# speedinghzl/CCNet

Measured on NVIDIA B200. Metric: cca_fwd_bwd_pixels_per_s, higher is better.
Workload: dtype f32

## Files before the change

ccnet_b200/csrc/cca_tc_bwd.cu:

```cuda
#include "cca_items.cuh"
#include "cca_tc_common.cuh"

namespace cca {
namespace {
using namespace tc;

constexpr int kTmemCols = 512;
constexpr int kTmemO = 256, kTmemQK = 384;
constexpr int kRegsSoft = 104, kRegsEpi = 128, kRegsConvB = 48;
static_assert(reg_pool_ok(kRegsSoft, kRegsEpi, kRegsConvB), "setmaxnreg pool");
constexpr int kZeroBuf = 2048;

struct BwdParams {
    ItemSpace sp;
    int C, Cq;
    long npix;
    const float *lse;
    float *delta;
    unsigned int *zdone;
    unsigned int *ddone;
    int delta_mode;
    int out_mode;
    unsigned int *cdone;
    int lag;
    int hints;
    uint8_t *dq, *dk, *dv;
    long sb_q, sb_v;
    long share_q, share_v;
    int ahead;
    long long *dbg;
};

#ifdef CCA_TIMELINE
#define CCA_STAMP(role)                                                                          \
    do {                                                                                         \
        if (p.dbg && blockIdx.x == 0 && dbg_n < 512) p.dbg[(role) * 512 + dbg_n++] = clock64();  \
    } while (0)
#else
#define CCA_STAMP(role) do { } while (0)
#endif

template <int LK, bool BF> struct BwdSmem {
    using T = Tiles<LK, BF>;
    static constexpr int kNLd = BF ? 6 : 5;
    static constexpr int off_ld = 0;
    static constexpr int kNOut = BF ? 3 : 1;
    static constexpr int off_out = off_ld + kNLd * T::kSlot;
    static constexpr int off_p = off_out + kNOut * T::kSlot;
    static constexpr int off_tail = off_p + T::kP + (16 - LK / 8) * T::kPlane;
    static constexpr int off_zero = off_tail + (128 - LK) * 16 + 256;
    static constexpr int off_dpart = off_zero + kZeroBuf;
    static constexpr int off_bar = off_dpart + 2048 + 32;
    static constexpr int kBytes = off_bar + 8 * 48 + 32;
    static_assert(kBytes <= 232448, "shared memory budget");
};

enum { B_LD_FULL = 0, B_LD_EMPTY = 6, B_OP_FULL = 12, B_S_FULL = 18, B_S_EMPTY = 20, B_P_FULL = 22,
       B_P_EMPTY = 23, B_O_FULL = 24, B_O_EMPTY = 26, B_OUT_FULL = 28, B_STAGED = 29, B_DP_FULL = 30, B_DS_FULL = 31,
       B_DELTA_FULL = 32, B_DELTA_EMPTY = 33, B_OUT_FREE = 34, B_STAGED_W = 37, B_QK_FULL = 43, B_QK_EMPTY = 45,
       B_COUNT = 47 };

__device__ __forceinline__ bool calc_delta(const BwdParams &p, const Item &it) { return p.delta_mode == 0 || (it.col && it.ik == 0); }

template <int LK, bool BF>
__device__ __forceinline__ float convert_dot(uint8_t *dslot, const uint8_t *oslot, int t, uint64_t *o_empty, unsigned int *o_cnt)
{
    using T = Tiles<LK, BF>;
    const int grp = t >> 8, r = t & 127, hq = (t >> 7) & 1;
    const int rr = r < LK ? r : LK - 1;
    const int sw = rr & 7;
    float acc = 0.f;
    auto group_sync_and_release = [&]() {
        if (grp == 0) asm volatile("bar.sync 1, 256;" ::: "memory");
        else asm volatile("bar.sync 3, 256;" ::: "memory");
        if ((t & 255) == 0 && atomicAdd(o_cnt, 1u) == 1u) {
            *o_cnt = 0u;
            mbar_arrive(o_empty);
        }
    };
    if constexpr (BF) {
        const uint8_t *a = dslot + rr * 128, *b = oslot + rr * 128;
#pragma unroll
        for (int i = 0; i < 2; ++i) {
            const int j = (grp * 2 + hq) * 2 + i;
            const uint4 x = *reinterpret_cast<const uint4 *>(a + ((j ^ sw) * 16));
            const uint4 y = *reinterpret_cast<const uint4 *>(b + ((j ^ sw) * 16));
            const uint32_t xw[4] = {x.x, x.y, x.z, x.w}, yw[4] = {y.x, y.y, y.z, y.w};
#pragma unroll
            for (int e = 0; e < 4; ++e) acc += bf_lo(xw[e]) * bf_lo(yw[e]) + bf_hi(xw[e]) * bf_hi(yw[e]);
        }
        group_sync_and_release();
    } else {
        float4 raw[4];
        uint8_t *box = dslot + grp * T::kTile;
        const uint8_t *src = box + rr * 128;
        const uint8_t *osrc = oslot + grp * T::kTile + rr * 128;
#pragma unroll
        for (int j = 0; j < 4; ++j) raw[j] = *reinterpret_cast<const float4 *>(src + (((hq * 4 + j) ^ sw) * 16));
#pragma unroll
        for (int j = 0; j < 4; ++j) {
            const float4 o = *reinterpret_cast<const float4 *>(osrc + (((hq * 4 + j) ^ sw) * 16));
            acc += raw[j].x * o.x + raw[j].y * o.y + raw[j].z * o.z + raw[j].w * o.w;
        }
        group_sync_and_release();
        if (r < LK) {
            uint8_t *d = box + r * 16 + hq * 2 * T::kPStride;
#pragma unroll
            for (int j = 0; j < 2; ++j) {
                const float4 a = raw[2 * j], b = raw[2 * j + 1];
                const float v[8] = {a.x, a.y, a.z, a.w, b.x, b.y, b.z, b.w};
                uint4 hi, lo;
                split8(v, hi, lo);
                *reinterpret_cast<uint4 *>(d + j * T::kPStride) = hi;
                *reinterpret_cast<uint4 *>(d + j * T::kPStride + T::kLoOff) = lo;
            }
        }
    }
    return acc;
}

template <int LK, bool BF>
__global__ void __launch_bounds__(kThreads, 1)
cca_tc_bwd_kernel(const __grid_constant__ CUtensorMap mqc, const __grid_constant__ CUtensorMap mqr,
                  const __grid_constant__ CUtensorMap mkc, const __grid_constant__ CUtensorMap mkr,
                  const __grid_constant__ CUtensorMap mvc, const __grid_constant__ CUtensorMap mvr,
                  const __grid_constant__ CUtensorMap mdoc, const __grid_constant__ CUtensorMap mdor,
                  const __grid_constant__ CUtensorMap moc, const __grid_constant__ CUtensorMap mor,
                  const __grid_constant__ CUtensorMap mdqc, const __grid_constant__ CUtensorMap mdqr,
                  const __grid_constant__ CUtensorMap mdkc, const __grid_constant__ CUtensorMap mdkr,
                  const __grid_constant__ CUtensorMap mdvc, const __grid_constant__ CUtensorMap mdvr, BwdParams p)
{
    using T = Tiles<LK, BF>;
    using S = BwdSmem<LK, BF>;
    constexpr int TERMS = BF ? 1 : 3;
    constexpr int kNLd = S::kNLd;
    constexpr int kNOut = S::kNOut;
    extern __shared__ __align__(1024) uint8_t smem[];
    uint64_t *bars = reinterpret_cast<uint64_t *>(smem + S::off_bar);
    uint32_t *tmem_slot = reinterpret_cast<uint32_t *>(smem + S::off_bar + 8 * B_COUNT);
    float *dpart = reinterpret_cast<float *>(smem + S::off_dpart);
    unsigned int *o_cnt = reinterpret_cast<unsigned int *>(smem + S::off_dpart + 2048);
    const int tid = threadIdx.x, warp = tid >> 5, lane = tid & 31;
    const int NCH = p.C / kNC;
    const int KQ = p.Cq / 16;
    const int NO = NCH + 2;
    const int nk = p.sp.total > (int)blockIdx.x ? (p.sp.total - (int)blockIdx.x + (int)gridDim.x - 1) / (int)gridDim.x : 0;
    auto item_of = [&](int k) { return decode_item_order(p.sp, (int)blockIdx.x + k * (int)gridDim.x, p.lag); };

    if (tid == 0) {
        for (int i = 0; i < kNLd; ++i) {
            mbar_init(&bars[B_LD_FULL + i], 1); mbar_init(&bars[B_LD_EMPTY + i], 1); mbar_init(&bars[B_OP_FULL + i], kConvThreads);
        }
        for (int i = 0; i < 2; ++i) { mbar_init(&bars[B_O_FULL + i], 1); mbar_init(&bars[B_O_EMPTY + i], 128); }
        for (int i = 0; i < 3; ++i) { mbar_init(&bars[B_OUT_FREE + i], 1); mbar_init(&bars[B_STAGED_W + i], 128); mbar_init(&bars[B_STAGED_W + 3 + i], 128); }
        for (int i = 0; i < 2; ++i) { mbar_init(&bars[B_S_FULL + i], 1); mbar_init(&bars[B_S_EMPTY + i], 128); }
        for (int i = 0; i < 2; ++i) { mbar_init(&bars[B_QK_FULL + i], 1); mbar_init(&bars[B_QK_EMPTY + i], 128); }
        mbar_init(&bars[B_P_FULL], 128); mbar_init(&bars[B_P_EMPTY], 1);
        mbar_init(&bars[B_DP_FULL], 1);  mbar_init(&bars[B_DS_FULL], 128);
        mbar_init(&bars[B_DELTA_FULL], kConvThreads); mbar_init(&bars[B_DELTA_EMPTY], 128);
        fence_mbar_init();
        prefetch_tmap(&mqc); prefetch_tmap(&mqr); prefetch_tmap(&mkc); prefetch_tmap(&mkr); prefetch_tmap(&mvc); prefetch_tmap(&mvr);
        prefetch_tmap(&mdoc); prefetch_tmap(&mdor); prefetch_tmap(&moc); prefetch_tmap(&mor);
        prefetch_tmap(&mdqc); prefetch_tmap(&mdqr); prefetch_tmap(&mdkc); prefetch_tmap(&mdkr); prefetch_tmap(&mdvc); prefetch_tmap(&mdvr);
    }
    if (tid < kZeroBuf / 16) {
        reinterpret_cast<uint4 *>(smem + S::off_zero)[tid] = make_uint4(0, 0, 0, 0);
        fence_proxy_async();
    }
    if (tid < 8) o_cnt[tid] = 0u;
    if (warp == 0) tmem_alloc<kTmemCols>(tmem_slot);
    tc_fence_before();
    __syncthreads();
    tc_fence_after();
    const uint32_t tmem = *tmem_slot;

    if (warp >= kWarpProducer) {
        reg_dec<kRegsMisc>();
        if (warp == kWarpProducer) {
            if (lane == 0) {
                uint32_t g = 0;
                int dbg_n = 0;
                (void)dbg_n;
                const uint64_t pol_keep = l2_policy_evict_last(), pol_stream = l2_policy_evict_first();
                auto emit = [&](const CUtensorMap *mc, const CUtensorMap *mr, int c0, const Item &it, int start, bool last_use = false) {
                    const CUtensorMap *m = it.col ? mc : mr;
                    const int cw = it.col ? it.line : start, ch = it.col ? start : it.line;
                    const int slot = g % kNLd;
                    mbar_wait(&bars[B_LD_EMPTY + slot], ((g / kNLd) & 1) ^ 1);
                    CCA_STAMP(0);
                    uint8_t *dst = smem + S::off_ld + slot * T::kSlot;
                    mbar_expect_tx(&bars[B_LD_FULL + slot], T::kSlot);
                    if (p.hints == 1) {
                        const uint64_t pol = (is_producer(it) && !last_use) ? pol_keep : pol_stream;
                        tma_load_4d(dst, m, &bars[B_LD_FULL + slot], c0, cw, ch, it.b, pol);
                        if constexpr (!BF) tma_load_4d(dst + T::kTile, m, &bars[B_LD_FULL + slot], c0 + 32, cw, ch, it.b, pol);
                    } else {
                        tma_load_4d(dst, m, &bars[B_LD_FULL + slot], c0, cw, ch, it.b);
                        if constexpr (!BF) tma_load_4d(dst + T::kTile, m, &bars[B_LD_FULL + slot], c0 + 32, cw, ch, it.b);
                    }
                    ++g;
                };
                if (nk > 0) {
                    const Item it0 = item_of(0);
                    emit(&mqc, &mqr, 0, it0, it0.q0);
                    emit(&mkc, &mkr, 0, it0, it0.k0);
                }
                for (int k = 0; k < nk; ++k) {
                    const Item it = item_of(k);
                    const bool calc = calc_delta(p, it);
                    for (int n = 0; n < NCH; ++n) {
                        emit(&mvc, &mvr, n * kNC, it, it.k0);
                        emit(&mdoc, &mdor, n * kNC, it, it.q0);
                        if (calc) emit(&moc, &mor, n * kNC, it, it.q0, p.delta_mode == 1);
                    }
                    if (k + 1 < nk) {
                        const Item nx = item_of(k + 1);
                        emit(&mqc, &mqr, 0, nx, nx.q0);
                        emit(&mkc, &mkr, 0, nx, nx.k0);
                    }
                    emit(&mqc, &mqr, 0, it, it.q0);
                    emit(&mkc, &mkr, 0, it, it.k0);
                }
            }
        } else if (warp == kWarpMma) {
            const uint32_t id_kk_s = instr_desc(kFmtBF16, kFmtBF16, 128, LK, false, false);
            const uint32_t id_mn_mn = instr_desc(kFmtBF16, kFmtBF16, 128, kNC, true, true);
            const uint32_t id_k_mn = instr_desc(kFmtBF16, kFmtBF16, 128, kNC, false, true);
            const uint32_t pb = smem_u32(smem + S::off_p);
            const uint32_t LO8 = BF ? 0 : T::kLoOff, LOP = T::kPP * T::kPlane;
            uint32_t u = 0, oc = 0;
            int dbg_n = lane == 0 ? 0 : 512;
            (void)dbg_n;
            const uint32_t ld_base = smem_u32(smem + S::off_ld);
            auto opb = [&](uint32_t g) { return ld_base + (g % kNLd) * T::kSlot; };
            auto wait_op = [&](uint32_t g) { mbar_wait(&bars[B_OP_FULL + g % kNLd], (g / kNLd) & 1); };
            auto free_op = [&](uint32_t g) { commit_to(&bars[B_LD_EMPTY + g % kNLd]); };
            constexpr uint32_t KS_K = BF ? 32 : 2 * T::kPStride, LBO_K = BF ? 16 : T::kPStride, SBO_K = BF ? 1024 : 128;
            constexpr uint32_t KS_MN = BF ? 2048 : 256, LBO_MN = BF ? 16 : 128, SBO_MN = BF ? 1024 : T::kPStride;
            constexpr uint32_t LAY = BF ? kSw128 : 0;
            auto issue_s = [&](int k) {
                const uint32_t q = opb(u), kk = opb(u + 1);
                wait_op(u); wait_op(u + 1);
                mbar_wait(&bars[B_S_EMPTY + (k & 1)], ((k >> 1) & 1) ^ 1);
                tc_fence_after();
                const uint32_t d = tmem + (k & 1) * 128;
                for (int ks = 0; ks < KQ; ++ks) {
                    const uint32_t ao = ks * KS_K;
                    mma_split3<TERMS>(d, smem_desc(q + ao, LBO_K, SBO_K, LAY), smem_desc(q + LO8 + ao, LBO_K, SBO_K, LAY),
                                      smem_desc(kk + ao, LBO_K, SBO_K, LAY), smem_desc(kk + LO8 + ao, LBO_K, SBO_K, LAY), id_kk_s, ks > 0);
                }
                commit_to(&bars[B_S_FULL + (k & 1)]);
                free_op(u); free_op(u + 1);
                u += 2;
            };
            if (nk > 0) issue_s(0);
            for (int k = 0; k < nk; ++k) {
                const bool calc = calc_delta(p, item_of(k));
                CCA_STAMP(2);
                const uint32_t sdp = tmem + (k & 1) * 128;
                mbar_wait(&bars[B_P_FULL], k & 1);
                CCA_STAMP(2);
                for (int n = 0; n < NCH; ++n, u += calc ? 3 : 2, ++oc) {
                    const uint32_t vb = opb(u), db = opb(u + 1);
                    wait_op(u); wait_op(u + 1);
                    tc_fence_after();
                    mma_split3_loop<kNC / 16, TERMS>(sdp, db, db + LO8, KS_K, LBO_K, SBO_K,
                                                     vb, vb + LO8, KS_K, LBO_K, SBO_K, id_kk_s, n > 0, LAY, LAY);
                    free_op(u);
                    mbar_wait(&bars[B_O_EMPTY + (oc & 1)], ((oc >> 1) & 1) ^ 1);
                    tc_fence_after();
                    mma_split3_loop<LK / 16, TERMS>(tmem + kTmemO + (oc & 1) * kNC, pb, pb + LOP, 256, 128, T::kPlane,
                                                    db, db + LO8, KS_MN, LBO_MN, SBO_MN, id_mn_mn, false, 0, LAY);
                    commit_to(&bars[B_O_FULL + (oc & 1)]);
                    free_op(u + 1);
                    CCA_STAMP(2);
                }
                commit_to(&bars[B_DP_FULL]);
                if (k + 1 < nk) issue_s(k + 1);
                mbar_wait(&bars[B_DS_FULL], k & 1);
                CCA_STAMP(2);
                {
                    const uint32_t q = opb(u), kk = opb(u + 1);
                    wait_op(u); wait_op(u + 1);
                    mbar_wait(&bars[B_QK_EMPTY + 0], (k & 1) ^ 1);
                    mbar_wait(&bars[B_QK_EMPTY + 1], (k & 1) ^ 1);
                    tc_fence_after();
                    mma_split3_loop<LK / 16, TERMS>(tmem + kTmemQK, pb, pb + LOP, 2 * T::kPlane, T::kPlane, 128,
                                                    kk, kk + LO8, KS_MN, LBO_MN, SBO_MN, id_k_mn, false, 0, LAY);
                    commit_to(&bars[B_QK_FULL + 0]);
                    free_op(u + 1);
                    mma_split3_loop<LK / 16, TERMS>(tmem + kTmemQK + kNC, pb, pb + LOP, 256, 128, T::kPlane,
                                                    q, q + LO8, KS_MN, LBO_MN, SBO_MN, id_mn_mn, false, 0, LAY);
                    commit_to(&bars[B_QK_FULL + 1]);
                    free_op(u);
                    commit_to(&bars[B_P_EMPTY]);
                    u += 2;
                }
                CCA_STAMP(2);
            }
        } else if (warp >= kWarpStore) {
            if (lane == 0) {
                pdl_wait();
                const uint64_t pol_keep = l2_policy_evict_last(), pol_stream = l2_policy_evict_first();
                int pending = -1;
                const int sel = warp - kWarpStore;
                uint32_t use[3] = {0, 0, 0};
                for (int k = sel; k < nk; k += 2) {
                    uint32_t c = (uint32_t)k * NO;
                    const Item it = item_of(k);
                    const bool prod = p.out_mode == 1 && is_producer(it);
                    const int zb = it.b + p.ahead;
                    if (p.out_mode == 0 && zb < p.sp.B) {
                        uint8_t *dst[3] = {p.dq + (long)zb * p.sb_q, p.dk + (long)zb * p.sb_q, p.dv + (long)zb * p.sb_v};
                        for (int t = 0; t < 3; ++t) {
                            const long sh = t < 2 ? p.share_q : p.share_v, sb = t < 2 ? p.sb_q : p.sb_v;
                            const long lo = (long)it.j * sh;
                            const long hi = lo + sh < sb ? lo + sh : sb;
                            for (long o = lo; o < hi; o += kZeroBuf)
                                bulk_store(dst[t] + o, smem + S::off_zero, (uint32_t)(hi - o < kZeroBuf ? hi - o : kZeroBuf));
                        }
                        tma_store_commit();
                        pending = zb;
                    }
                    for (int i = 0; i < NO; ++i, ++c) {
                        const CUtensorMap *m = i < NCH ? (it.col ? &mdvc : &mdvr) : (i == NCH ? (it.col ? &mdqc : &mdqr) : (it.col ? &mdkc : &mdkr));
                        const int c0 = i < NCH ? i * kNC : 0;
                        const int start = i == NCH ? it.q0 : it.k0;
                        const int cw = it.col ? it.line : start, ch = it.col ? start : it.line;
                        const int os = c % kNOut;
                        uint8_t *slot = smem + S::off_out + os * T::kSlot;
                        mbar_wait(&bars[B_STAGED_W + sel * 3 + os], use[os] & 1);
                        ++use[os];
                        if (i == 0) {
                            if (pending >= 0) {
                                tma_store_wait_all<0>();
                                publish_count(p.zdone + pending);
                                pending = -1;
                            }
                            if (p.out_mode == 0 && it.b >= p.ahead) {
                                wait_count(p.zdone + it.b, (unsigned)p.sp.per_sample);
                                fence_proxy_async_all();
                            }
                            if (p.out_mode == 1 && !prod) {
                                wait_count(p.cdone + it.b, (unsigned)p.sp.seg0);
                                fence_proxy_async_all();
                            }
                        }
                        if (prod) {
                            if (p.hints) {
                                tma_store_4d(m, slot, c0, cw, ch, it.b, pol_keep);
                                if constexpr (!BF) tma_store_4d(m, slot + T::kTile, c0 + 32, cw, ch, it.b, pol_keep);
                            } else {
                                tma_store_4d(m, slot, c0, cw, ch, it.b);
                                if constexpr (!BF) tma_store_4d(m, slot + T::kTile, c0 + 32, cw, ch, it.b);
                            }
                        } else if (p.hints && p.out_mode == 1) {
                            tma_reduce_add_4d(m, slot, c0, cw, ch, it.b, pol_stream);
                            if constexpr (!BF) tma_reduce_add_4d(m, slot + T::kTile, c0 + 32, cw, ch, it.b, pol_stream);
                        } else {
                            tma_reduce_add_4d(m, slot, c0, cw, ch, it.b);
                            if constexpr (!BF) tma_reduce_add_4d(m, slot + T::kTile, c0 + 32, cw, ch, it.b);
                        }
                        tma_store_commit();
                        tma_store_wait_read<0>();
                        mbar_arrive(&bars[B_OUT_FREE + os]);
                    }
                    if (prod) {
                        tma_store_wait_all<0>();
                        publish_count(p.cdone + it.b);
                    }
                }
                tma_store_wait_all<0>();
                if (pending >= 0) publish_count(p.zdone + pending);
            }
        }
    } else if (warp >= kWarpConv0) {
        reg_dec<kRegsConvB>();
        const int t = tid - kWarpConv0 * 32;
        int dbg_n = t == 0 ? 0 : 512;
        (void)dbg_n;
        uint32_t g = 0, ncalc = 0;
        uint32_t pend = 0;
        auto publish = [&]() {
            if (pend) {
                if constexpr (!BF) fence_proxy_async();
                for (int sl = 0; sl < kNLd; ++sl)
                    if (pend & (1u << sl)) mbar_arrive(&bars[B_OP_FULL + sl]);
                pend = 0;
            }
        };
        auto wait_full = [&](uint32_t gg) {
            const int slot = gg % kNLd;
            if (!mbar_try_wait(&bars[B_LD_FULL + slot], (gg / kNLd) & 1)) {
                publish();
                mbar_wait(&bars[B_LD_FULL + slot], (gg / kNLd) & 1);
            }
        };
        auto conv = [&](int count) {
            for (int e = 0; e < count; ++e, ++g) {
                const int slot = g % kNLd;
                wait_full(g);
                CCA_STAMP(1);
                if constexpr (!BF) {
                    convert_slot_inplace<LK>(smem + S::off_ld + slot * T::kSlot, t);
                    pend |= 1u << slot;
                    publish();
                } else {
                    mbar_arrive(&bars[B_OP_FULL + slot]);
                }
                CCA_STAMP(1);
            }
        };
        if (nk > 0) conv(2);
        for (int k = 0; k < nk; ++k) {
            const bool calc = calc_delta(p, item_of(k));
            float dacc = 0.f;
            for (int n = 0; n < NCH; ++n) {
                conv(1);
                if (calc) {
                    const int sd = g % kNLd, so = (g + 1) % kNLd;
                    wait_full(g);
                    wait_full(g + 1);
                    publish();
                    dacc += convert_dot<LK, BF>(smem + S::off_ld + sd * T::kSlot, smem + S::off_ld + so * T::kSlot, t, &bars[B_LD_EMPTY + so],
                                                o_cnt + so);
                    if constexpr (!BF) {
                        pend |= (1u << sd) | (1u << so);
                        publish();
                    } else {
                        mbar_arrive(&bars[B_OP_FULL + sd]);
                        mbar_arrive(&bars[B_OP_FULL + so]);
                    }
                    g += 2;
                } else {
                    conv(1);
                }
            }
            if (calc) {
                publish();
                mbar_wait(&bars[B_DELTA_EMPTY], (ncalc & 1) ^ 1);
                dpart[(t >> 7) * 128 + (t & 127)] = dacc;
                mbar_arrive(&bars[B_DELTA_FULL]);
                ++ncalc;
            }
            if (k + 1 < nk) conv(2);
            conv(2);
        }
        publish();
    } else if (warp >= 4) {
        reg_inc<kRegsSoft>();
        const int r = tid - 128;
        const uint32_t tl = tmem + ((uint32_t)((warp & 3) * 32) << 16);
        int dbg_n = r == 0 ? 0 : 512;
        (void)dbg_n;
        uint32_t ncalc = 0;
        pdl_wait();
        for (int k = 0; k < nk; ++k) {
            const Item it = item_of(k);
            const bool calc = calc_delta(p, it);
            const bool rvalid = r < it.lq;
            const long pix = item_pixel(p.sp, it, rvalid ? r : 0);
            const float nlse = rvalid ? -p.lse[pix] * kLog2e : -INFINITY;
            const int self = it.col ? it.q0 + r - it.k0 : -1;
            const int sw0 = it.col ? it.q0 - it.k0 + 32 * (warp & 3) : -(1 << 20);
            uint8_t *ph = smem + S::off_p + r * 16, *pl = ph + T::kPP * T::kPlane;
            const uint32_t tsd = tl + (k & 1) * 128;
            CCA_STAMP(3);
            mbar_wait(&bars[B_S_FULL + (k & 1)], (k >> 1) & 1);
            tc_fence_after();
            CCA_STAMP(3);
            float nx[16];
            tmem_ld16(tsd, reinterpret_cast<uint32_t *>(nx));
            mbar_wait(&bars[B_P_EMPTY], (k & 1) ^ 1);
#pragma unroll
            for (int c0 = 0; c0 < LK; c0 += 16) {
                float s[16];
                tmem_ld_wait16(reinterpret_cast<uint32_t *>(nx));
#pragma unroll
                for (int e = 0; e < 16; ++e) s[e] = nx[e];
                if (c0 + 16 < LK) tmem_ld16(tsd + c0 + 16, reinterpret_cast<uint32_t *>(nx));
                if (!((c0 + 16 > it.lk) || (c0 + 16 > sw0 && c0 < sw0 + 32))) {
#pragma unroll
                    for (int e = 0; e < 16; ++e) s[e] = exp2f(fmaf(s[e], kLog2e, nlse));
                } else {
#pragma unroll
                    for (int e = 0; e < 16; ++e) {
                        const int j = c0 + e;
                        s[e] = (j < it.lk && j != self) ? exp2f(fmaf(s[e], kLog2e, nlse)) : 0.f;
                    }
                }
                if (r < LK) {
#pragma unroll
                    for (int h = 0; h < 2; ++h) {
                        const int kc = c0 / 8 + h;
                        const float *v8 = s + h * 8;
                        if constexpr (BF) {
                            *reinterpret_cast<uint4 *>(ph + kc * T::kPlane) =
                                make_uint4(pack_bf16(v8[0], v8[1]), pack_bf16(v8[2], v8[3]), pack_bf16(v8[4], v8[5]), pack_bf16(v8[6], v8[7]));
                        } else {
                            uint4 hi, lo;
                            split8(v8, hi, lo);
                            *reinterpret_cast<uint4 *>(ph + kc * T::kPlane) = hi;
                            *reinterpret_cast<uint4 *>(pl + kc * T::kPlane) = lo;
                        }
                    }
                }
            }
            tc_fence_before();
            fence_proxy_async();
            mbar_arrive(&bars[B_P_FULL]);
            CCA_STAMP(3);
            float dl = 0.f;
            if (calc) {
                mbar_wait(&bars[B_DELTA_FULL], ncalc & 1);
                dl = (dpart[r] + dpart[128 + r]) + (dpart[256 + r] + dpart[384 + r]);
                mbar_arrive(&bars[B_DELTA_EMPTY]);
                ++ncalc;
                if (rvalid && is_producer(it)) p.delta[pix] = dl;
                if (p.delta_mode == 1) {
                    named_bar_sync(2, 128);
                    if (r == 0) { __threadfence(); atomicAdd(p.ddone + it.b, 1u); }
                }
            } else {
                wait_count(p.ddone + it.b, (unsigned)p.sp.seg0);
                if (rvalid) dl = __ldcg(p.delta + pix);
            }
            mbar_wait(&bars[B_DP_FULL], k & 1);
            tc_fence_after();
            CCA_STAMP(3);
            tmem_ld16(tsd, reinterpret_cast<uint32_t *>(nx));
#pragma unroll
            for (int c0 = 0; c0 < LK; c0 += 16) {
                float dp[16];
                tmem_ld_wait16(reinterpret_cast<uint32_t *>(nx));
#pragma unroll
                for (int e = 0; e < 16; ++e) dp[e] = nx[e];
                if (c0 + 16 < LK) tmem_ld16(tsd + c0 + 16, reinterpret_cast<uint32_t *>(nx));
                if (r < LK) {
#pragma unroll
                    for (int h = 0; h < 2; ++h) {
                        const int kc = c0 / 8 + h;
                        const uint4 hi = *reinterpret_cast<const uint4 *>(ph + kc * T::kPlane);
                        uint4 lo = make_uint4(0, 0, 0, 0);
                        if constexpr (!BF) lo = *reinterpret_cast<const uint4 *>(pl + kc * T::kPlane);
                        const uint32_t hw[4] = {hi.x, hi.y, hi.z, hi.w}, lw[4] = {lo.x, lo.y, lo.z, lo.w};
                        float ds[8];
#pragma unroll
                        for (int e = 0; e < 4; ++e) {
                            const float p0 = bf_lo(hw[e]) + bf_lo(lw[e]), p1 = bf_hi(hw[e]) + bf_hi(lw[e]);
                            ds[2 * e] = p0 * (dp[h * 8 + 2 * e] - dl);
                            ds[2 * e + 1] = p1 * (dp[h * 8 + 2 * e + 1] - dl);
                        }
                        if constexpr (BF) {
                            *reinterpret_cast<uint4 *>(ph + kc * T::kPlane) =
                                make_uint4(pack_bf16(ds[0], ds[1]), pack_bf16(ds[2], ds[3]), pack_bf16(ds[4], ds[5]), pack_bf16(ds[6], ds[7]));
                        } else {
                            uint4 dh, dlo;
                            split8(ds, dh, dlo);
                            *reinterpret_cast<uint4 *>(ph + kc * T::kPlane) = dh;
                            *reinterpret_cast<uint4 *>(pl + kc * T::kPlane) = dlo;
                        }
                    }
                }
            }
            tc_fence_before();
            mbar_arrive(&bars[B_S_EMPTY + (k & 1)]);
            fence_proxy_async();
            mbar_arrive(&bars[B_DS_FULL]);
            CCA_STAMP(3);
        }
    } else {
        reg_inc<kRegsEpi>();
        const int r = tid;
        const uint32_t tl = tmem + ((uint32_t)(warp * 32) << 16);
        uint32_t oc = 0, nt = 0;
        int dbg_n = tid == 0 ? 0 : 512;
        (void)dbg_n;
        for (int k = 0; k < nk; ++k) {
            for (int i = 0; i < NO; ++i, ++nt) {
                const bool qk = i >= NCH;
                const int ob = oc & 1;
                const int os = nt % kNOut;
                uint8_t *slot = smem + S::off_out + os * T::kSlot;
                CCA_STAMP(4);
                mbar_wait(&bars[B_OUT_FREE + os], ((nt / kNOut) & 1) ^ 1);
                if (qk) mbar_wait(&bars[B_QK_FULL + (i - NCH)], k & 1);
                else mbar_wait(&bars[B_O_FULL + ob], (oc >> 1) & 1);
                tc_fence_after();
                CCA_STAMP(4);
                float o[kNC];
                const uint32_t src = tl + (qk ? kTmemQK + (i - NCH) * kNC : kTmemO + ob * kNC);
#pragma unroll
                for (int c0 = 0; c0 < kNC; c0 += 16) tmem_ld16(src + c0, reinterpret_cast<uint32_t *>(o + c0));
                tmem_ld_wait();
                tc_fence_before();
                if (qk) mbar_arrive(&bars[B_QK_EMPTY + (i - NCH)]);
                else { mbar_arrive(&bars[B_O_EMPTY + ob]); ++oc; }
                if (r < LK) {
                    uint8_t *row = slot + r * 128;
                    const int sw = r & 7;
                    if constexpr (BF) {
#pragma unroll
                        for (int j = 0; j < 8; ++j)
                            *reinterpret_cast<uint4 *>(row + ((j ^ sw) * 16)) =
                                make_uint4(pack_bf16(o[8 * j], o[8 * j + 1]), pack_bf16(o[8 * j + 2], o[8 * j + 3]),
                                           pack_bf16(o[8 * j + 4], o[8 * j + 5]), pack_bf16(o[8 * j + 6], o[8 * j + 7]));
                    } else {
#pragma unroll
                        for (int j = 0; j < 16; ++j)
                            *reinterpret_cast<float4 *>(row + (j >> 3) * T::kTile + (((j & 7) ^ sw) * 16)) =
                                make_float4(o[4 * j], o[4 * j + 1], o[4 * j + 2], o[4 * j + 3]);
                    }
                }
                fence_proxy_async();
                mbar_arrive(&bars[B_STAGED_W + (k & 1) * 3 + os]);
                CCA_STAMP(4);
            }
        }
    }
    tc_fence_before();
    __syncthreads();
    if (warp == 0) tmem_dealloc<kTmemCols>(tmem);
}

__global__ void __launch_bounds__(256) cca_bwd_prep_kernel(uint4 *dq, uint4 *dk, uint4 *dv, long nq16, long nv16,
                                                           unsigned int *counters, int n_counters)
{
    pdl_launch_dependents();
    const long tid = (long)blockIdx.x * blockDim.x + threadIdx.x, nth = (long)gridDim.x * blockDim.x;
    const uint4 z = make_uint4(0, 0, 0, 0);
    for (long i = tid; i < nq16; i += nth) { dq[i] = z; dk[i] = z; }
    for (long i = tid; i < nv16; i += nth) dv[i] = z;
    for (long i = tid; i < n_counters; i += nth) counters[i] = 0u;
}

long long *g_bwd_dbg = nullptr;

template <int LK, bool BF>
cudaError_t launch_bwd(const void *dout, const void *q, const void *k, const void *v, const void *out, const float *lse, float *delta,
                       unsigned int *counters, void *dq, void *dk, void *dv, Dims d, int ahead, int delta_mode, cudaStream_t st,
                       const char **why)
{
    CUtensorMap m[16];
    const void *base[8] = {q, k, v, dout, out, dq, dk, dv};
    const int ch[8] = {d.Cq, d.Cq, d.C, d.C, d.C, d.Cq, d.Cq, d.C};
    BwdParams p;
    p.sp = make_space(d.B, d.H, d.W);
    for (int t = 0; t < 8; ++t)
        for (int r = 0; r < 2; ++r) {
            const int rows = t < 5 ? LK : (r == 0 ? p.sp.col.tl : p.sp.row.tl);
            if (!get_map(&m[2 * t + r], base[t], d.B, d.H, d.W, ch[t], rows, r == 0, BF)) {
                if (why) *why = "cuTensorMapEncodeTiled failed";
                return cudaErrorInvalidValue;
            }
        }
    p.C = d.C; p.Cq = d.Cq;
    p.npix = (long)d.B * d.H * d.W;
    p.lse = lse; p.delta = delta;
    p.zdone = counters; p.ddone = counters + d.B; p.cdone = counters + 2 * d.B;
    p.delta_mode = delta_mode;
    const bool one_tile = p.sp.col.nt == 1 && p.sp.row.nt == 1;
    p.out_mode = one_tile ? 1 : 0;
    p.lag = (p.out_mode == 1 && tc_lag() != 0) ? 1 : 0;
    p.hints = tc_l2_hints();
    p.dq = reinterpret_cast<uint8_t *>(dq); p.dk = reinterpret_cast<uint8_t *>(dk); p.dv = reinterpret_cast<uint8_t *>(dv);
    const long es = BF ? 2 : 4;
    p.sb_q = (long)d.H * d.W * d.Cq * es; p.sb_v = (long)d.H * d.W * d.C * es;
    p.share_q = zero_share_bytes(p.sb_q, p.sp.per_sample); p.share_v = zero_share_bytes(p.sb_v, p.sp.per_sample);
    p.ahead = ahead;
    p.dbg = g_bwd_dbg;
    const int head = p.out_mode == 1 ? 0 : (ahead < d.B ? ahead : d.B);
    cca_bwd_prep_kernel<<<p.out_mode == 1 ? 1 : sm_count(), 256, 0, st>>>(
        reinterpret_cast<uint4 *>(dq), reinterpret_cast<uint4 *>(dk), reinterpret_cast<uint4 *>(dv), head * p.sb_q / 16,
        head * p.sb_v / 16, counters, 3 * d.B);
    count_launch();
    cudaError_t e = cudaGetLastError();
    if (e != cudaSuccess) return e;
    auto kern = cca_tc_bwd_kernel<LK, BF>;
    e = cudaFuncSetAttribute(kern, cudaFuncAttributeMaxDynamicSharedMemorySize, BwdSmem<LK, BF>::kBytes);
    if (e != cudaSuccess) return e;
    const int sms = sm_count();
    const int grid = p.sp.total < sms ? p.sp.total : sms;
    cudaLaunchConfig_t cfg = {};
    cfg.gridDim = dim3(grid); cfg.blockDim = dim3(kThreads); cfg.dynamicSmemBytes = BwdSmem<LK, BF>::kBytes; cfg.stream = st;
    cudaLaunchAttribute attr[1];
    attr[0].id = cudaLaunchAttributeProgrammaticStreamSerialization;
    attr[0].val.programmaticStreamSerializationAllowed = 1;
    cfg.attrs = attr;
    cfg.numAttrs = tc_pdl() ? 1 : 0;
    e = cudaLaunchKernelEx(&cfg, kern, m[0], m[1], m[2], m[3], m[4], m[5], m[6], m[7], m[8], m[9], m[10], m[11], m[12], m[13],
                           m[14], m[15], p);
    count_launch();
    return e != cudaSuccess ? e : cudaGetLastError();
}

}

void set_tc_bwd_debug_buffer(void *p) { g_bwd_dbg = reinterpret_cast<long long *>(p); }

bool tc_backward_supported(Dims d, int dtype) { return tc::shape_supported(d, dtype); }

size_t tc_backward_workspace(Dims d)
{
    const size_t delta = ((size_t)d.B * d.H * d.W * sizeof(float) + 15) & ~(size_t)15;
    return delta + (((size_t)3 * d.B * sizeof(unsigned int) + 15) & ~(size_t)15);
}

cudaError_t tc_backward(const void *dout, const void *q, const void *k, const void *v, const void *out, const float *lse,
                        void *dq, void *dk, void *dv, void *ws, Dims d, int dtype, cudaStream_t st, const char **why)
{
    float *delta = reinterpret_cast<float *>(ws);
    const size_t delta_bytes = ((size_t)d.B * d.H * d.W * sizeof(float) + 15) & ~(size_t)15;
    unsigned int *counters = reinterpret_cast<unsigned int *>(reinterpret_cast<uint8_t *>(ws) + delta_bytes);
    const ItemSpace sp = make_space(d.B, d.H, d.W);
    const int lk = lk_for(max_tile(sp));
    const bool bf = dtype == CCA_BF16;
    int ahead = tc_zero_ahead();
    if (ahead < 1) ahead = 1;
    int mode = tc_delta_mode();
    if (mode < 0) mode = 1;
    if (bf)
        return lk == 80 ? launch_bwd<80, true>(dout, q, k, v, out, lse, delta, counters, dq, dk, dv, d, ahead, mode, st, why)
                        : launch_bwd<112, true>(dout, q, k, v, out, lse, delta, counters, dq, dk, dv, d, ahead, mode, st, why);
    return lk == 80 ? launch_bwd<80, false>(dout, q, k, v, out, lse, delta, counters, dq, dk, dv, d, ahead, mode, st, why)
                    : launch_bwd<112, false>(dout, q, k, v, out, lse, delta, counters, dq, dk, dv, d, ahead, mode, st, why);
}

}
```

Measured before the change: 88.40 million.

## Compute transposed probabilities in TMEM via extra S^T MMA for dV

Adds a second MMA that computes the transposed score tile S^T into TMEM. The epilogue warps turn it into probabilities P^T (exp2 with the stored negative LSE, masking, bf16 or split packing) and write them back to TMEM, so the dV MMA can read its A operand from TMEM instead of the shared-memory P buffer. The dQ/dK accumulators now reuse the S/dP TMEM regions with double-buffered barriers, which frees columns and lets the epilogue lag one item behind. The cost is duplicated QK^T MMA work and exp work, plus more complex barrier phasing that could add stalls.

```diff
diff --git a/ccnet_b200/csrc/cca_tc_bwd.cu b/ccnet_b200/csrc/cca_tc_bwd.cu
--- a/ccnet_b200/csrc/cca_tc_bwd.cu
+++ b/ccnet_b200/csrc/cca_tc_bwd.cu
@@ -6,7 +6,7 @@
 using namespace tc;
 
 constexpr int kTmemCols = 512;
-constexpr int kTmemO = 256, kTmemQK = 384;
+constexpr int kTmemPT = 256, kTmemO = 384;
 constexpr int kRegsSoft = 104, kRegsEpi = 128, kRegsConvB = 48;
 static_assert(reg_pool_ok(kRegsSoft, kRegsEpi, kRegsConvB), "setmaxnreg pool");
 constexpr int kZeroBuf = 2048;
@@ -50,14 +50,15 @@
     static constexpr int off_tail = off_p + T::kP + (16 - LK / 8) * T::kPlane;
     static constexpr int off_zero = off_tail + (128 - LK) * 16 + 256;
     static constexpr int off_dpart = off_zero + kZeroBuf;
-    static constexpr int off_bar = off_dpart + 2048 + 32;
+    static constexpr int off_nlse = off_dpart + 2048 + 32;
+    static constexpr int off_bar = off_nlse + 2 * 128 * 4;
     static constexpr int kBytes = off_bar + 8 * 48 + 32;
     static_assert(kBytes <= 232448, "shared memory budget");
 };
 
-enum { B_LD_FULL = 0, B_LD_EMPTY = 6, B_OP_FULL = 12, B_S_FULL = 18, B_S_EMPTY = 20, B_P_FULL = 22,
-       B_P_EMPTY = 23, B_O_FULL = 24, B_O_EMPTY = 26, B_OUT_FULL = 28, B_STAGED = 29, B_DP_FULL = 30, B_DS_FULL = 31,
-       B_DELTA_FULL = 32, B_DELTA_EMPTY = 33, B_OUT_FREE = 34, B_STAGED_W = 37, B_QK_FULL = 43, B_QK_EMPTY = 45,
+enum { B_LD_FULL = 0, B_LD_EMPTY = 6, B_OP_FULL = 12, B_S_FULL = 18, B_ST_FULL = 20, B_PT_FULL = 21, B_P_FULL = 22,
+       B_P_EMPTY = 23, B_O_FULL = 24, B_O_EMPTY = 26, B_QK_EMPTY = 28, B_DP_FULL = 30, B_DS_FULL = 31,
+       B_DELTA_FULL = 32, B_DELTA_EMPTY = 33, B_OUT_FREE = 34, B_STAGED_W = 37, B_QK_FULL = 43,
        B_COUNT = 47 };
 
 __device__ __forceinline__ bool calc_delta(const BwdParams &p, const Item &it) { return p.delta_mode == 0 || (it.col && it.ik == 0); }
@@ -153,8 +154,10 @@
         }
         for (int i = 0; i < 2; ++i) { mbar_init(&bars[B_O_FULL + i], 1); mbar_init(&bars[B_O_EMPTY + i], 128); }
         for (int i = 0; i < 3; ++i) { mbar_init(&bars[B_OUT_FREE + i], 1); mbar_init(&bars[B_STAGED_W + i], 128); mbar_init(&bars[B_STAGED_W + 3 + i], 128); }
-        for (int i = 0; i < 2; ++i) { mbar_init(&bars[B_S_FULL + i], 1); mbar_init(&bars[B_S_EMPTY + i], 128); }
-        for (int i = 0; i < 2; ++i) { mbar_init(&bars[B_QK_FULL + i], 1); mbar_init(&bars[B_QK_EMPTY + i], 128); }
+        for (int i = 0; i < 2; ++i) mbar_init(&bars[B_S_FULL + i], 1);
+        mbar_init(&bars[B_ST_FULL], 1); mbar_init(&bars[B_PT_FULL], 128);
+        for (int i = 0; i < 4; ++i) mbar_init(&bars[B_QK_FULL + i], 1);
+        for (int i = 0; i < 2; ++i) mbar_init(&bars[B_QK_EMPTY + i], 128);
         mbar_init(&bars[B_P_FULL], 128); mbar_init(&bars[B_P_EMPTY], 1);
         mbar_init(&bars[B_DP_FULL], 1);  mbar_init(&bars[B_DS_FULL], 128);
         mbar_init(&bars[B_DELTA_FULL], kConvThreads); mbar_init(&bars[B_DELTA_EMPTY], 128);
@@ -238,10 +241,12 @@
             constexpr uint32_t KS_K = BF ? 32 : 2 * T::kPStride, LBO_K = BF ? 16 : T::kPStride, SBO_K = BF ? 1024 : 128;
             constexpr uint32_t KS_MN = BF ? 2048 : 256, LBO_MN = BF ? 16 : 128, SBO_MN = BF ? 1024 : T::kPStride;
             constexpr uint32_t LAY = BF ? kSw128 : 0;
+            const uint32_t tpt = tmem + kTmemPT;
+            uint32_t oc_last = 0;
             auto issue_s = [&](int k) {
                 const uint32_t q = opb(u), kk = opb(u + 1);
                 wait_op(u); wait_op(u + 1);
-                mbar_wait(&bars[B_S_EMPTY + (k & 1)], ((k >> 1) & 1) ^ 1);
+                mbar_wait(&bars[B_QK_EMPTY + (k & 1)], ((k >> 1) & 1) ^ 1);
                 tc_fence_after();
                 const uint32_t d = tmem + (k & 1) * 128;
                 for (int ks = 0; ks < KQ; ++ks) {
@@ -250,6 +255,16 @@
                                       smem_desc(kk + ao, LBO_K, SBO_K, LAY), smem_desc(kk + LO8 + ao, LBO_K, SBO_K, LAY), id_kk_s, ks > 0);
                 }
                 commit_to(&bars[B_S_FULL + (k & 1)]);
+                if (k > 0) {
+                    mbar_wait(&bars[B_O_FULL + (oc_last & 1)], (oc_last >> 1) & 1);
+                    tc_fence_after();
+                }
+                for (int ks = 0; ks < KQ; ++ks) {
+                    const uint32_t ao = ks * KS_K;
+                    mma_split3<TERMS>(tpt, smem_desc(kk + ao, LBO_K, SBO_K, LAY), smem_desc(kk + LO8 + ao, LBO_K, SBO_K, LAY),
+                                      smem_desc(q + ao, LBO_K, SBO_K, LAY), smem_desc(q + LO8 + ao, LBO_K, SBO_K, LAY), id_kk_s, ks > 0);
+                }
+                commit_to(&bars[B_ST_FULL]);
                 free_op(u); free_op(u + 1);
                 u += 2;
             };
@@ -267,12 +282,26 @@
                     mma_split3_loop<kNC / 16, TERMS>(sdp, db, db + LO8, KS_K, LBO_K, SBO_K,
                                                      vb, vb + LO8, KS_K, LBO_K, SBO_K, id_kk_s, n > 0, LAY, LAY);
                     free_op(u);
+                    if (n == 0) mbar_wait(&bars[B_PT_FULL], k & 1);
                     mbar_wait(&bars[B_O_EMPTY + (oc & 1)], ((oc >> 1) & 1) ^ 1);
                     tc_fence_after();
-                    mma_split3_loop<LK / 16, TERMS>(tmem + kTmemO + (oc & 1) * kNC, pb, pb + LOP, 256, 128, T::kPlane,
-                                                    db, db + LO8, KS_MN, LBO_MN, SBO_MN, id_mn_mn, false, 0, LAY);
+                    if (elect_one()) {
+                        const uint32_t d = tmem + kTmemO + (oc & 1) * kNC;
+#pragma unroll
+                        for (int ks = 0; ks < LK / 16; ++ks) {
+                            const uint32_t ph = tpt + ks * 16;
+                            const uint64_t bh = smem_desc(db + ks * KS_MN, LBO_MN, SBO_MN, LAY);
+                            mma_f16_ts(d, ph, bh, id_k_mn, ks > 0);
+                            if constexpr (TERMS == 3) {
+                                mma_f16_ts(d, ph, smem_desc(db + LO8 + ks * KS_MN, LBO_MN, SBO_MN, LAY), id_k_mn, true);
+                                mma_f16_ts(d, ph + 8, bh, id_k_mn, true);
+                            }
+                        }
+                    }
+                    __syncwarp();
                     commit_to(&bars[B_O_FULL + (oc & 1)]);
                     free_op(u + 1);
+                    oc_last = oc;
                     CCA_STAMP(2);
                 }
                 commit_to(&bars[B_DP_FULL]);
@@ -282,16 +311,14 @@
                 {
                     const uint32_t q = opb(u), kk = opb(u + 1);
                     wait_op(u); wait_op(u + 1);
-                    mbar_wait(&bars[B_QK_EMPTY + 0], (k & 1) ^ 1);
-                    mbar_wait(&bars[B_QK_EMPTY + 1], (k & 1) ^ 1);
                     tc_fence_after();
-                    mma_split3_loop<LK / 16, TERMS>(tmem + kTmemQK, pb, pb + LOP, 2 * T::kPlane, T::kPlane, 128,
+                    mma_split3_loop<LK / 16, TERMS>(sdp, pb, pb + LOP, 2 * T::kPlane, T::kPlane, 128,
                                                     kk, kk + LO8, KS_MN, LBO_MN, SBO_MN, id_k_mn, false, 0, LAY);
-                    commit_to(&bars[B_QK_FULL + 0]);
+                    commit_to(&bars[B_QK_FULL + 2 * (k & 1)]);
                     free_op(u + 1);
-                    mma_split3_loop<LK / 16, TERMS>(tmem + kTmemQK + kNC, pb, pb + LOP, 256, 128, T::kPlane,
+                    mma_split3_loop<LK / 16, TERMS>(sdp + kNC, pb, pb + LOP, 256, 128, T::kPlane,
                                                     q, q + LO8, KS_MN, LBO_MN, SBO_MN, id_mn_mn, false, 0, LAY);
-                    commit_to(&bars[B_QK_FULL + 1]);
+                    commit_to(&bars[B_QK_FULL + 2 * (k & 1) + 1]);
                     free_op(u);
                     commit_to(&bars[B_P_EMPTY]);
                     u += 2;
@@ -507,7 +534,6 @@
                 }
             }
             tc_fence_before();
-            fence_proxy_async();
             mbar_arrive(&bars[B_P_FULL]);
             CCA_STAMP(3);
             float dl = 0.f;
@@ -564,7 +590,6 @@
                 }
             }
             tc_fence_before();
-            mbar_arrive(&bars[B_S_EMPTY + (k & 1)]);
             fence_proxy_async();
             mbar_arrive(&bars[B_DS_FULL]);
             CCA_STAMP(3);
@@ -573,29 +598,93 @@
         reg_inc<kRegsEpi>();
         const int r = tid;
         const uint32_t tl = tmem + ((uint32_t)(warp * 32) << 16);
-        uint32_t oc = 0, nt = 0;
+        const uint32_t tpt = tl + kTmemPT;
+        uint32_t oc = 0;
         int dbg_n = tid == 0 ? 0 : 512;
         (void)dbg_n;
-        for (int k = 0; k < nk; ++k) {
-            for (int i = 0; i < NO; ++i, ++nt) {
+        pdl_wait();
+        auto compute_pt = [&](int k) {
+            const Item it = item_of(k);
+            float *nl = reinterpret_cast<float *>(smem + S::off_nlse) + (k & 1) * 128;
+            nl[r] = r < it.lq ? -p.lse[item_pixel(p.sp, it, r)] * kLog2e : -INFINITY;
+            named_bar_sync(4, 128);
+            const int self = it.col ? it.k0 + r - it.q0 : -1;
+            const int sw0 = it.col ? it.k0 - it.q0 + 32 * warp : -(1 << 20);
+            mbar_wait(&bars[B_ST_FULL], k & 1);
+            tc_fence_after();
+            CCA_STAMP(4);
+            float nx[16];
+            tmem_ld16(tpt, reinterpret_cast<uint32_t *>(nx));
+#pragma unroll
+            for (int c0 = 0; c0 < LK; c0 += 16) {
+                float s[16];
+                tmem_ld_wait16(reinterpret_cast<uint32_t *>(nx));
+#pragma unroll
+                for (int e = 0; e < 16; ++e) s[e] = nx[e];
+                if (c0 + 16 < LK) tmem_ld16(tpt + c0 + 16, reinterpret_cast<uint32_t *>(nx));
+                float l[16];
+#pragma unroll
+                for (int e = 0; e < 4; ++e) {
+                    const float4 v = reinterpret_cast<const float4 *>(nl + c0)[e];
+                    l[4 * e] = v.x; l[4 * e + 1] = v.y; l[4 * e + 2] = v.z; l[4 * e + 3] = v.w;
+                }
+                uint32_t hi[8], lo[8];
+                if (!((c0 + 16 > it.lq) || (c0 + 16 > sw0 && c0 < sw0 + 32))) {
+#pragma unroll
+                    for (int e = 0; e < 8; ++e) {
+                        const float p0 = exp2f(fmaf(s[2 * e], kLog2e, l[2 * e]));
+                        const float p1 = exp2f(fmaf(s[2 * e + 1], kLog2e, l[2 * e + 1]));
+                        if constexpr (BF) hi[e] = pack_bf16(p0, p1);
+                        else split2(p0, p1, hi[e], lo[e]);
+                    }
+                } else {
+#pragma unroll
+                    for (int e = 0; e < 8; ++e) {
+                        const int j = c0 + 2 * e;
+                        const bool ok0 = j < it.lq && j != self;
+                        const bool ok1 = j + 1 < it.lq && j + 1 != self;
+                        const float p0 = ok0 ? exp2f(fmaf(s[2 * e], kLog2e, l[2 * e])) : 0.f;
+                        const float p1 = ok1 ? exp2f(fmaf(s[2 * e + 1], kLog2e, l[2 * e + 1])) : 0.f;
+                        if constexpr (BF) hi[e] = pack_bf16(p0, p1);
+                        else split2(p0, p1, hi[e], lo[e]);
+                    }
+                }
+                if (r >= it.lk) {
+#pragma unroll
+                    for (int e = 0; e < 8; ++e) { hi[e] = 0u; lo[e] = 0u; }
+                }
+                tmem_st8(tpt + c0, hi);
+                if constexpr (!BF) tmem_st8(tpt + c0 + 8, lo);
+            }
+            tmem_st_wait();
+            tc_fence_before();
+            mbar_arrive(&bars[B_PT_FULL]);
+            CCA_STAMP(4);
+        };
+        for (int j = 0; j <= nk; ++j) {
+            if (j < nk) compute_pt(j);
+            for (int t = j > 0 ? 0 : 2; t < (j < nk ? NO : 2); ++t) {
+                const int k = t < 2 ? j - 1 : j;
+                const int i = t < 2 ? NCH + t : t - 2;
+                const uint32_t nt = (uint32_t)k * NO + i;
                 const bool qk = i >= NCH;
                 const int ob = oc & 1;
                 const int os = nt % kNOut;
                 uint8_t *slot = smem + S::off_out + os * T::kSlot;
                 CCA_STAMP(4);
                 mbar_wait(&bars[B_OUT_FREE + os], ((nt / kNOut) & 1) ^ 1);
-                if (qk) mbar_wait(&bars[B_QK_FULL + (i - NCH)], k & 1);
+                if (qk) mbar_wait(&bars[B_QK_FULL + 2 * (k & 1) + (i - NCH)], (k >> 1) & 1);
                 else mbar_wait(&bars[B_O_FULL + ob], (oc >> 1) & 1);
                 tc_fence_after();
                 CCA_STAMP(4);
                 float o[kNC];
-                const uint32_t src = tl + (qk ? kTmemQK + (i - NCH) * kNC : kTmemO + ob * kNC);
+                const uint32_t src = tl + (qk ? (k & 1) * 128 + (i - NCH) * kNC : kTmemO + ob * kNC);
 #pragma unroll
                 for (int c0 = 0; c0 < kNC; c0 += 16) tmem_ld16(src + c0, reinterpret_cast<uint32_t *>(o + c0));
                 tmem_ld_wait();
                 tc_fence_before();
-                if (qk) mbar_arrive(&bars[B_QK_EMPTY + (i - NCH)]);
-                else { mbar_arrive(&bars[B_O_EMPTY + ob]); ++oc; }
+                if (i == NCH + 1) mbar_arrive(&bars[B_QK_EMPTY + (k & 1)]);
+                else if (!qk) { mbar_arrive(&bars[B_O_EMPTY + ob]); ++oc; }
                 if (r < LK) {
                     uint8_t *row = slot + r * 128;
                     const int sw = r & 7;
```

Result: slower. 83.35 million (median of 6 runs) (-5.7%).
